# SKA-INAF/caesar-mrcnn

Measured on AMD Instinct MI355X. Metric: train images/sec (whole node) + detect ms/image, ResNet-101 256x256, higher is better.
Workload: dtype f32; 1 GPU; resnet101+FPN 256x256 3-class (+bg), nimg_per_gpu=4, train step (fwd+bwd+SGD), 512 train ROIs, 2000 proposals; global_batch=4, parallelism=dp1, weights=random init (Keras defaults)

## Files before the change

### caesar-mrcnn_amd/_hip.py

```python
import ctypes as C
import os
import threading

PKG_DIR = os.path.dirname(os.path.abspath(__file__))
LIB_PATH = os.path.join(PKG_DIR, "libmrcnn_hip.so")


class HipPathError(RuntimeError):
    pass


class ConvDesc(C.Structure):
    _fields_ = [(n, C.c_int32) for n in (
        "N", "H", "W", "Cin", "Cout", "KH", "KW", "stride", "pad_t", "pad_l", "OH", "OW",
        "act", "res_mode", "out_mode", "cmod")] + [
        ("out_n_stride", C.c_int64), ("out_h_stride", C.c_int64), ("out_w_stride", C.c_int64)]


class ConvProblem(C.Structure):
    _fields_ = [("d", ConvDesc)] + [(n, C.c_void_p) for n in ("x", "w", "bias", "scale", "shift", "res", "out", "z_out")]


class WgradProblem(C.Structure):
    _fields_ = [("d", ConvDesc), ("x", C.c_void_p), ("dy", C.c_void_p), ("dw", C.c_void_p), ("accumulate", C.c_int32)]
# ... 151 lines not shown
    "mrcnn_detection_targets": (C.c_int, [C.POINTER(DetTargetDesc)] + [_P] * 12),
    "mrcnn_conv2d_fwd_h16": (C.c_int, [C.POINTER(ConvDesc), C.c_int] + [_P] * 8),
    "mrcnn_conv2d_fwd_h16_res": (C.c_int, [C.POINTER(ConvDesc), C.c_int] + [_P] * 9),
    "mrcnn_conv2d_fwd_h16_supported": (C.c_int, [C.POINTER(ConvDesc), C.c_int]),
    "mrcnn_conv2d_dgrad_ep_h16": (C.c_int, [C.POINTER(ConvDesc), C.c_int, _P, _P, _P, _P, C.POINTER(BwdEpilogueH16), _P]),
    "mrcnn_conv2d_dgrad_ep": (C.c_int, [C.POINTER(ConvDesc), _P, _P, _P, _P, C.POINTER(BwdEpilogue), _P, C.c_size_t, _P]),
    "mrcnn_conv2d_wgrad_h16_workspace": (C.c_size_t, [C.POINTER(ConvDesc)]),
    "mrcnn_conv2d_wgrad_h16": (C.c_int, [C.POINTER(ConvDesc), C.c_int, _P, _P, _P, _P, C.c_size_t, C.c_int, C.c_float, _P]),
    "mrcnn_mask_out_fwd_h16": (C.c_int, [C.c_int, _P, _P, _P, _P, C.c_int64, C.c_int, C.c_int, _P]),
    "mrcnn_mask_out_bwd_h16": (C.c_int, [C.c_int] + [_P] * 8 + [C.c_int64, C.c_int, C.c_int, C.c_int, C.c_int, C.c_float, _P]),
    "mrcnn_weights_to_h16": (C.c_int, [_P, _P, _P, C.c_int, C.c_int, C.c_int, C.c_int, C.c_int, _P]),
    "mrcnn_weights_to_h16_batched": (C.c_int, [_P, _P, C.c_int, C.c_int, C.c_int, _P]),
    "mrcnn_cast_to_h16": (C.c_int, [_P, _P, C.c_int64, C.c_int, C.c_float, _P]),
    "mrcnn_epilogue_bwd_h16": (C.c_int, [C.c_int] + [_P] * 10 + [C.c_int64, C.c_int, C.c_int, C.c_float, _P]),
    "mrcnn_epilogue_bwd_h16_dy": (C.c_int, [C.c_int] + [_P] * 11 + [C.c_int64, C.c_int, C.c_int, C.c_float, _P]),
    "mrcnn_cast_from_h16": (C.c_int, [_P, _P, C.c_int64, C.c_int, C.c_float, _P]),
    "mrcnn_axpy_from_h16": (C.c_int, [_P, _P, C.c_int64, C.c_int, C.c_float, _P]),
    "mrcnn_rpn_targets_workspace": (C.c_size_t, [C.POINTER(RpnTargetDesc)]),
    "mrcnn_rpn_targets": (C.c_int, [C.POINTER(RpnTargetDesc)] + [_P] * 7 + [C.c_size_t, _P]),
    "mrcnn_detection_workspace": (C.c_size_t, [C.POINTER(DetectionDesc)]),
    "mrcnn_detection_fwd": (C.c_int, [C.POINTER(DetectionDesc)] + [_P] * 6 + [C.c_size_t, _P]),
    "mrcnn_losses_workspace": (C.c_size_t, [C.POINTER(LossDesc)]),
    "mrcnn_losses_fwd_bwd": (C.c_int, [C.POINTER(LossDesc)] + [_P] * 18 + [C.c_size_t, _P]),
    "mrcnn_grad_prepare": (C.c_int, [_P, _P, C.c_float, _P, C.c_int64, _P, _P]),
    "mrcnn_sumsq": (C.c_int, [_P, C.c_int64, _P, _P]),
    "mrcnn_sgd_momentum": (C.c_int, [_P, _P, _P, _P, C.c_float, C.c_float, C.c_float, _P, C.c_int64, _P]),
    "mrcnn_sgd_momentum_guarded": (C.c_int, [_P, _P, _P, _P, C.c_float, C.c_float, C.c_float, _P, C.c_int64, _P, _P]),
    "mrcnn_winograd_buffer_floats": (C.c_size_t, [C.c_int, C.c_int, C.c_int, C.c_int, C.c_int]),
    "mrcnn_winograd_weights": (C.c_int, [_P, _P, C.c_int, C.c_int, C.c_int, _P]),
    "mrcnn_gemm_batched_f32": (C.c_int, [_P, _P, _P, C.c_int, C.c_int, C.c_int, C.c_int, _P]),
    "mrcnn_winograd_gemm": (C.c_int, [_P, _P, _P, C.c_int, C.c_int, C.c_int, C.c_int, _P]),
    "mrcnn_winograd_group_floats": (C.c_size_t, [C.POINTER(WinoGroup), C.c_int, C.c_int]),
    "mrcnn_winograd_input_g": (C.c_int, [_P, _P, C.c_int, C.c_int, C.c_int, C.c_int, C.POINTER(WinoGroup), _P]),
    "mrcnn_winograd_weights_g": (C.c_int, [_P, _P, C.c_int, C.c_int, C.c_int, C.c_int, _P]),
    "mrcnn_winograd_output_g": (C.c_int, [_P, _P, _P, _P, _P, _P, C.c_int, C.c_int, C.c_int, C.c_int, C.c_int, C.POINTER(WinoGroup), _P]),
    "mrcnn_winograd_output_bwd_rows": (C.c_int, [C.POINTER(WinoGroup), C.c_int, C.c_int]),
    "mrcnn_winograd_output_bwd_g": (C.c_int, [_P] * 8 + [C.c_int, C.c_int, C.c_int, C.c_int, C.c_int, C.POINTER(WinoGroup), _P]),
    "mrcnn_winograd_output_bwd_zmask_g": (C.c_int, [_P] * 8 + [C.c_int, C.c_int, C.c_int, C.c_int, C.POINTER(WinoGroup), _P]),
    "mrcnn_winograd_output_bwd_sums": (C.c_int, [_P, C.c_int, C.c_int, _P, _P, _P, _P]),
    "mrcnn_winograd_dy_g": (C.c_int, [_P, _P, C.c_int, C.c_int, C.c_int, C.c_int, C.POINTER(WinoGroup), _P]),
    "mrcnn_winograd_dw_g": (C.c_int, [_P, _P, C.c_int, C.c_int, C.c_int, C.c_int, C.c_int, _P]),
    "mrcnn_deconv2x2_gemm": (C.c_int, [_P, _P, _P, _P, C.c_int, C.c_int, C.c_int, C.c_int, C.c_int, C.c_int, _P]),
    "mrcnn_allreduce_load": (C.c_int, [C.c_char_p]),
    "mrcnn_allreduce_unique_id": (C.c_int, [_P]),
    "mrcnn_allreduce_init": (C.c_int, [C.POINTER(_P), _P, C.c_int, C.c_int]),
    "mrcnn_allreduce_scratch": (C.c_size_t, [C.c_int, C.c_int64, C.c_int]),
    "mrcnn_allreduce_grad": (C.c_int, [_P, _P, C.c_int64, C.c_int64, C.c_int, _P, C.c_size_t, _P]),
    "mrcnn_allreduce_direct_plan": (C.c_int, [C.c_int, C.c_int, C.c_int64, C.c_int64, C.c_int, _P, _P, _P, _P]),
    "mrcnn_allreduce_direct_simulate": (C.c_int, [_P, _P, C.c_size_t, C.c_int, C.c_int64, C.c_int64, _P]),
    "mrcnn_allreduce_destroy": (C.c_int, [_P]),
    "mrcnn_allreduce_last_error": (C.c_char_p, []),
    "mrcnn_tuning_set": (C.c_int, [C.c_char_p, C.c_longlong]),
    "mrcnn_hip_version": (C.c_char_p, []),
}

_lib = None
_proxy = None
_tape = None
_tape_owner = None

_NO_RECORD = ("_workspace", "_fwd_plan", "_tiles_check", "_outline_check", "_draw_check", "_components_check", "_catalog_check", "_overview_check", "_planes_check", "_stats_check", "_gather_check", "_supported", "_status_offset", "_version", "mrcnn_allreduce_", "_scratch", "_floats", "_bwd_rows")


class _LibProxy(object):

    def __init__(self, real):
# ... 111 lines not shown
```

### caesar-mrcnn_amd/csrc/winograd.hip

```cpp
#include "common.h"
#include <type_traits>
#include <string.h>

template <int CV> struct WinoVec;
template <> struct WinoVec<4> { typedef f32x4 type; };
template <> struct WinoVec<2> { typedef float type __attribute__((ext_vector_type(2))); };

template <int OT, typename V> __device__ __forceinline__ void wino_bt(const V (&d)[OT + 2], V (&t)[OT + 2]) {
    if constexpr (OT == 2) {
        t[0] = d[0] - d[2];
        t[1] = d[1] + d[2];
        t[2] = d[2] - d[1];
        t[3] = d[1] - d[3];
    } else {
        const V a = d[4] - 4.f * d[2], b = d[3] - 4.f * d[1], c = d[4] - d[2], e = 2.f * (d[3] - d[1]);
        t[0] = 4.f * d[0] - 5.f * d[2] + d[4];
        t[1] = a + b;
        t[2] = a - b;
        t[3] = c + e;
        t[4] = c - e;
        t[5] = 4.f * d[1] - 5.f * d[3] + d[5];
    }
}
template <int OT, typename V> __device__ __forceinline__ void wino_at(const V (&m)[OT + 2], V (&y)[OT]) {
// ... 35 lines not shown
        u[0] = 0.25f * g[0];
        u[1] = (-1.f / 6.f) * (e + g[1]);
        u[2] = (-1.f / 6.f) * (e - g[1]);
        const float f = (1.f / 24.f) * g[0] + (1.f / 6.f) * g[2], h = (1.f / 12.f) * g[1];
        u[3] = f + h;
        u[4] = f - h;
        u[5] = g[2];
    }
}
template <int OT> __device__ __forceinline__ void wino_gt(const float (&u)[OT + 2], float (&w)[3]) {
    if constexpr (OT == 2) {
        w[0] = u[0] + 0.5f * (u[1] + u[2]);
        w[1] = 0.5f * (u[1] - u[2]);
        w[2] = 0.5f * (u[1] + u[2]) + u[3];
    } else {
        const float p = u[1] + u[2], q = u[3] + u[4];
        w[0] = 0.25f * u[0] - (1.f / 6.f) * p + (1.f / 24.f) * q;
        w[1] = (1.f / 6.f) * (u[2] - u[1]) + (1.f / 12.f) * (u[3] - u[4]);
        w[2] = (1.f / 6.f) * (q - p) + u[5];
    }
}

struct WinoGrp { int th_n, tw_n, oh0, ow0; };
struct WinoTile { int n, th, tw; };
__device__ __forceinline__ WinoTile wino_tile(long long t, int th_n, int tw_n) {
    WinoTile r;
    r.tw = (int)(t % tw_n);
    const long long q = t / tw_n;
    r.th = (int)(q % th_n);
    r.n = (int)(q / th_n);
    return r;
}

template <int OTH, int OTW, int CV>
__global__ __launch_bounds__(256) void winograd_input_kernel(const float* __restrict__ x, float* __restrict__ V, int N, int H, int W,
                                                             int C, long long T, long long Tp, const WinoGrp g) {
    typedef typename WinoVec<CV>::type vec;
    constexpr int ITH = OTH + 2, ITW = OTW + 2;
    const int cn = C / CV;
    const long long i = (long long)blockIdx.x * 256 + threadIdx.x;
    if (i >= T * cn) return;
    const long long t = i / cn;
    const int c = (int)(i - t * cn) * CV;
    const WinoTile q = wino_tile(t, g.th_n, g.tw_n);
    const int ih0 = g.oh0 + OTH * q.th - 1, iw0 = g.ow0 + OTW * q.tw - 1;
    vec tt[ITH][ITW];
#pragma unroll
    for (int s = 0; s < ITW; ++s) {
        vec col[ITH], o[ITH];
#pragma unroll
        for (int r = 0; r < ITH; ++r) {
            const int ih = ih0 + r, iw = iw0 + s;
            vec val = {};
            if ((unsigned)ih < (unsigned)H && (unsigned)iw < (unsigned)W) val = *(const vec*)(x + (((long long)q.n * H + ih) * W + iw) * C + c);
            col[r] = val;
        }
        wino_bt<OTH>(col, o);
#pragma unroll
        for (int r = 0; r < ITH; ++r) tt[r][s] = o[r];
    }
#pragma unroll
    for (int r = 0; r < ITH; ++r) {
        vec v[ITW];
        wino_bt<OTW>(tt[r], v);
#pragma unroll
        for (int s = 0; s < ITW; ++s) *(vec*)(V + ((long long)(r * ITW + s) * Tp + t) * C + c) = v[s];
    }
}

template <int OTH, int OTW>
__global__ __launch_bounds__(256) void winograd_weight_kernel(const float* __restrict__ g, float* __restrict__ U, int Cin, int Cout) {
    constexpr int ITH = OTH + 2, ITW = OTW + 2;
    const long long i = (long long)blockIdx.x * 256 + threadIdx.x;
    const long long n = (long long)Cin * Cout;
    if (i >= n) return;
    float t[ITH][3];
#pragma unroll
    for (int b = 0; b < 3; ++b) {
        float col[3], o[ITH];
#pragma unroll
        for (int a = 0; a < 3; ++a) col[a] = g[(long long)(a * 3 + b) * n + i];
        wino_g<OTH>(col, o);
#pragma unroll
        for (int a = 0; a < ITH; ++a) t[a][b] = o[a];
    }
#pragma unroll
    for (int a = 0; a < ITH; ++a) {
        float u[ITW];
        wino_g<OTW>(t[a], u);
#pragma unroll
        for (int b = 0; b < ITW; ++b) U[(long long)(a * ITW + b) * n + i] = u[b];
    }
}

template <int OTH, int OTW, int CV>
__device__ __forceinline__ void wino_output_tile(const float* __restrict__ Mt, float* __restrict__ out, float* __restrict__ z,
                                                 const typename WinoVec<CV>::type bi, const typename WinoVec<CV>::type sc,
                                                 const typename WinoVec<CV>::type sh, int H, int W, int C, long long Tp, int act,
                                                 const WinoGrp& g, long long t, int c) {
    typedef typename WinoVec<CV>::type vec;
    constexpr int ITH = OTH + 2, ITW = OTW + 2;
    const WinoTile q = wino_tile(t, g.th_n, g.tw_n);
    vec s[OTH][ITW];
#pragma unroll
    for (int k = 0; k < ITW; ++k) {
        vec col[ITH], o[OTH];
#pragma unroll
        for (int r = 0; r < ITH; ++r) col[r] = *(const vec*)(Mt + ((long long)(r * ITW + k) * Tp + t) * C + c);
        wino_at<OTH>(col, o);
#pragma unroll
        for (int a = 0; a < OTH; ++a) s[a][k] = o[a];
    }
#pragma unroll
    for (int a = 0; a < OTH; ++a) {
        vec y[OTW];
        wino_at<OTW>(s[a], y);
        const int oh = g.oh0 + OTH * q.th + a;
        if (oh >= H) continue;
#pragma unroll
        for (int b = 0; b < OTW; ++b) {
            const int ow = g.ow0 + OTW * q.tw + b;
            if (ow >= W) continue;
            const long long addr = (((long long)q.n * H + oh) * W + ow) * C + c;
            vec zv, o;
#pragma unroll
            for (int e = 0; e < CV; ++e) {
                zv[e] = y[b][e] + bi[e];
                float v = sc[e] * zv[e] + sh[e];
                if (act == MRCNN_ACT_RELU) v = fmaxf(v, 0.f);
                o[e] = v;
            }
            if (z) *(vec*)(z + addr) = zv;
            *(vec*)(out + addr) = o;
        }
    }
}

template <int OTH, int OTW, int CV>
__global__ __launch_bounds__(256) void winograd_output_kernel(const float* __restrict__ Mt, float* __restrict__ out, float* __restrict__ z,
                                                              const float* __restrict__ bias, const float* __restrict__ scale,
                                                              const float* __restrict__ shift, int N, int H, int W, int C, long long T,
                                                              long long Tp, int act, const WinoGrp g) {
    typedef typename WinoVec<CV>::type vec;
    const int cn = C / CV;
    const long long i = (long long)blockIdx.x * 256 + threadIdx.x;
    if (i >= T * cn) return;
    const long long t = i / cn;
    const int c = (int)(i - t * cn) * CV;
    vec bi = {}, sc, sh = {};
#pragma unroll
    for (int e = 0; e < CV; ++e) sc[e] = 1.f;
    if (bias) bi = *(const vec*)(bias + c);
    if (scale) { sc = *(const vec*)(scale + c); sh = *(const vec*)(shift + c); }
    wino_output_tile<OTH, OTW, CV>(Mt, out, z, bi, sc, sh, H, W, C, Tp, act, g, t, c);
}

template <int CV>
__device__ __forceinline__ typename WinoVec<CV>::type wino_buffer_load(__amdgpu_buffer_rsrc_t rsrc, unsigned voff, unsigned soff) {
    typename WinoVec<CV>::type r;
    if constexpr (CV == 2) {
        const auto v = __builtin_amdgcn_raw_buffer_load_b64(rsrc, (int)voff, (int)soff, 0);
        r[0] = __uint_as_float(v[0]); r[1] = __uint_as_float(v[1]);
    } else {
        const auto v = __builtin_amdgcn_raw_buffer_load_b128(rsrc, (int)voff, (int)soff, 0);
        r[0] = __uint_as_float(v[0]); r[1] = __uint_as_float(v[1]); r[2] = __uint_as_float(v[2]); r[3] = __uint_as_float(v[3]);
    }
// ... 367 lines not shown
static inline long long wino_grp_tiles(const mrcnn_wino_group* g, int N) { return (long long)N * g->th_n * g->tw_n; }
static inline int wino_grp_nb(const mrcnn_wino_group* g) { return (g->oth + 2) * (g->otw + 2); }
static inline int wino_grp_cv(const mrcnn_wino_group* g) { return g->oth == 2 && g->otw == 2 ? 4 : 2; }

#define WINO_LAUNCH_G(kernel, g, grid4, grid2, ...)                                                                          \
    do {                                                                                                                     \
        if ((g)->oth == 2 && (g)->otw == 2) hipLaunchKernelGGL((kernel<2, 2, 4>), grid4, dim3(256), 0, (hipStream_t)stream, __VA_ARGS__); \
        else if ((g)->oth == 4 && (g)->otw == 4) hipLaunchKernelGGL((kernel<4, 4, 2>), grid2, dim3(256), 0, (hipStream_t)stream, __VA_ARGS__); \
        else if ((g)->oth == 4) hipLaunchKernelGGL((kernel<4, 2, 2>), grid2, dim3(256), 0, (hipStream_t)stream, __VA_ARGS__); \
        else hipLaunchKernelGGL((kernel<2, 4, 2>), grid2, dim3(256), 0, (hipStream_t)stream, __VA_ARGS__);                  \
    } while (0)
#define WINO_LAUNCH_W(kernel, oth, otw, grid, ...)                                                                           \
    do {                                                                                                                     \
        if ((oth) == 2 && (otw) == 2) hipLaunchKernelGGL((kernel<2, 2>), grid, dim3(256), 0, (hipStream_t)stream, __VA_ARGS__); \
        else if ((oth) == 4 && (otw) == 4) hipLaunchKernelGGL((kernel<4, 4>), grid, dim3(256), 0, (hipStream_t)stream, __VA_ARGS__); \
        else if ((oth) == 4) hipLaunchKernelGGL((kernel<4, 2>), grid, dim3(256), 0, (hipStream_t)stream, __VA_ARGS__);     \
        else hipLaunchKernelGGL((kernel<2, 4>), grid, dim3(256), 0, (hipStream_t)stream, __VA_ARGS__);                     \
    } while (0)

extern "C" size_t mrcnn_winograd_group_floats(const mrcnn_wino_group* g, int N, int C) {
    if (!g || N <= 0 || C <= 0 || (g->oth != 2 && g->oth != 4) || (g->otw != 2 && g->otw != 4) || g->th_n <= 0 || g->tw_n <= 0) return 0;
    return (size_t)wino_grp_nb(g) * (size_t)wino_rows(wino_grp_tiles(g, N)) * (size_t)C;
}

extern "C" int mrcnn_winograd_input_g(const float* x, float* V, int N, int H, int W, int C, const mrcnn_wino_group* g, void* stream) {
    if (!x || !V || !wino_grp_ok(g, N, H, W, C)) return MRCNN_ERR_ARG;
    const long long T = wino_grp_tiles(g, N);
    const WinoGrp k = {g->th_n, g->tw_n, g->oh0, g->ow0};
    const dim3 g4((unsigned)cdiv64(T * C / 4, 256)), g2((unsigned)cdiv64(T * C / 2, 256));
    WINO_LAUNCH_G(winograd_input_kernel, g, g4, g2, x, V, N, H, W, C, T, wino_rows(T), k);
    return mrcnn_launch_status();
}

extern "C" int mrcnn_winograd_weights_g(const float* w, float* U, int Cin, int Cout, int oth, int otw, void* stream) {
    if (!w || !U || Cin <= 0 || Cout <= 0 || (oth != 2 && oth != 4) || (otw != 2 && otw != 4)) return MRCNN_ERR_ARG;
    const dim3 grid((unsigned)cdiv64((long long)Cin * Cout, 256));
    WINO_LAUNCH_W(winograd_weight_kernel, oth, otw, grid, w, U, Cin, Cout);
    return mrcnn_launch_status();
}

extern "C" int mrcnn_winograd_output_g(const float* Mt, float* out, float* z, const float* bias, const float* scale, const float* shift,
                                       int N, int H, int W, int C, int act, const mrcnn_wino_group* g, void* stream) {
    if (!Mt || !out || !wino_grp_ok(g, N, H, W, C) || (scale && !shift)) return MRCNN_ERR_ARG;
    if (act != MRCNN_ACT_NONE && act != MRCNN_ACT_RELU) return MRCNN_ERR_UNSUPPORTED;
    const long long T = wino_grp_tiles(g, N);
    const WinoGrp k = {g->th_n, g->tw_n, g->oh0, g->ow0};
    const dim3 g4((unsigned)cdiv64(T * C / 4, 256)), g2((unsigned)cdiv64(T * C / 2, 256));
    WINO_LAUNCH_G(winograd_output_kernel, g, g4, g2, Mt, out, z, bias, scale, shift, N, H, W, C, T, wino_rows(T), act, k);
    return mrcnn_launch_status();
}

static int wino_bwd_lanes_lg(const mrcnn_wino_group* g, int C) {
    const int cn = C / wino_grp_cv(g);
    if (cn <= 0 || cn > 256 || (cn & (cn - 1)) || cn * wino_grp_cv(g) != C) return -1;
    int lg = 0;
    while ((1 << lg) < cn) ++lg;
    return lg;
}
extern "C" int mrcnn_winograd_output_bwd_rows(const mrcnn_wino_group* g, int N, int C) {
    if (!g || N <= 0 || (g->oth != 2 && g->oth != 4) || (g->otw != 2 && g->otw != 4) || g->th_n <= 0 || g->tw_n <= 0) return 0;
    const int lg = wino_bwd_lanes_lg(g, C);
    if (lg < 0) return 0;
    const long long T = wino_grp_tiles(g, N), R = 256 >> lg, cap = 4LL * mrcnn_num_cus();
    const long long wgs = cdiv64(T, R);
    return (int)(wgs < cap ? wgs : cap);
}

template <int MASK>
static int wino_output_bwd_launch(const float* Mt, float* dz_below, const float* below_out, const float* below_z, const float* scale,
                                  const float* mean, const float* rstd, const float* fwd_shift, float* partials, int N, int H, int W,
                                  int C, const mrcnn_wino_group* g, void* stream) {
    const int lg = wino_bwd_lanes_lg(g, C);
    const long long T = wino_grp_tiles(g, N);
    if (lg < 0) return MRCNN_ERR_UNSUPPORTED;
    if ((long long)wino_grp_nb(g) * wino_rows(T) * C * 4 >= (1LL << 32) || (long long)N * H * W * C * 4 >= (1LL << 32)) return MRCNN_ERR_UNSUPPORTED;
    const dim3 grid((unsigned)mrcnn_winograd_output_bwd_rows(g, N, C));
// ... 112 lines not shown
```

### caesar-mrcnn_amd/engine.py

```python
import collections
import contextlib
import gc
import operator
from functools import partial
import os
import numpy as np
import torch

from . import ops
from . import _hip as _hip_mod
from ._hip import ACT_NONE, ACT_RELU, ACT_SIGMOID, RES_NONE, RES_SAME, RES_UP2
from .params import ParamLayout, deconv_gemm_to_keras, deconv_keras_to_gemm, granule_coefficients, init_weights

H16_WIDE_LAYERS = ("fpn_p2", "fpn_p3", "fpn_p4", "fpn_p5", "rpn_conv_shared", "mrcnn_class_conv1", "mrcnn_class_conv2")

LOSS_NAMES = ("rpn_class_loss", "rpn_bbox_loss", "mrcnn_class_loss", "mrcnn_bbox_loss", "mrcnn_mask_loss")


DIRECT, WINO, H16 = "direct", "winograd", "h16"
Ctx = collections.namedtuple("Ctx", "x z out act path V", defaults=(DIRECT, None))
BlockCtx = collections.namedtuple("BlockCtx", "a b c shortcut h16")


_on = lambda s: s != "0"

SWITCHES = (
    ("head_dtype", None, None, None, "ti"),
    ("sparse_mask_bwd", None, True, None, "t"),
    ("h16_wide", "MRCNN_H16_WIDE", True, _on, "ti"),
    ("h16_blocks", "MRCNN_H16_BLOCKS", True, _on, "ti"),
    ("h16_all_blocks", "MRCNN_H16_ALL_BLOCKS", True, _on, "ti"),
    ("h16_fused_bwd", "MRCNN_H16_FUSED_BWD", True, _on, "t"),
    ("h16_roialign", "MRCNN_H16_ROIALIGN", True, _on, "ti"),
    ("h16_phase_bwd", "MRCNN_H16_PHASE_BWD", True, _on, "t"),
    ("winograd", "MRCNN_WINOGRAD", True, _on, "ti"),
    ("winograd_wgrad", "MRCNN_WINOGRAD_WGRAD", True, _on, "t"),
    ("trunk_winograd", "MRCNN_WINOGRAD_TRUNK", True, _on, "ti"),
    ("trunk_winograd_min_rows", "MRCNN_WINOGRAD_TRUNK_MIN_ROWS", 4096, int, "ti"),
    ("infer_mask_tile", "MRCNN_WINOGRAD_INFER_MASK_TILE", 4, int, "i"),
    ("sk16_infer", "MRCNN_SK16_INFER", True, _on, "i"),
    ("fused_mask_out_bwd", None, True, None, "t"),
    ("fused_dgrad_epilogue", None, True, None, "t"),
    ("gather_roialign_bwd", "MRCNN_GATHER_ROIALIGN_BWD", True, _on, "t"),
    ("multi_launch", "MRCNN_MULTI_LAUNCH", True, _on, "ti"),
    ("wgrad_prio", "MRCNN_WGRAD_PRIO", 0, int, ""),
    ("aux_prio", "MRCNN_AUX_PRIO", 0, int, ""),
)
_TRAIN_SWITCHES = operator.attrgetter(*(s[0] for s in SWITCHES if "t" in s[4]))
_INFER_SWITCHES = operator.attrgetter(*(s[0] for s in SWITCHES if "i" in s[4]))
_INFER_CFG = operator.attrgetter("PRE_NMS_LIMIT", "POST_NMS_ROIS_INFERENCE", "RPN_NMS_THRESHOLD", "DETECTION_MAX_INSTANCES",
                                 "DETECTION_MIN_CONFIDENCE", "DETECTION_NMS_THRESHOLD")


@contextlib.contextmanager
def _capture(graph):
    gc.collect()
    was = gc.isenabled()
    gc.disable()
    try:
        with torch.cuda.graph(graph):
            yield
    finally:
        if was:
            gc.enable()


@contextlib.contextmanager
def _tuning(key, value, restore, on=True):
    if on:
        ops.tuning_set(key, value)
    try:
        yield
    finally:
        if on:
            ops.tuning_set(key, restore)
# ... 354 lines not shown
                return got
        d = self._h16_dgrad(op, dz)
        return ops.epilogue_bwd_h16(d, y if act != ACT_NONE else None, z, below.scale, below.mean, below.rstd, below.dgamma,
                                    below.dbeta, below.db, act, 1.0 / S)

    def _block_bwd_h16(self, blk, d16, ctxs, S):
        ca, cb, cc, c1c = ctxs.a, ctxs.b, ctxs.c, ctxs.shortcut
        c2a, c2b, c2c = blk.c2a, blk.c2b, blk.c2c
        dzc, dy = ops.epilogue_bwd_h16(d16, cc.out, cc.z, c2c.scale, c2c.mean, c2c.rstd, c2c.dgamma, c2c.dbeta, c2c.db, ACT_RELU,
                                       1.0 / S, want_dy=True)
        self._h16_wgrad(c2c, cc.x, dzc, S)
        dzb = self._h16_dgrad_ep(c2c, dzc, c2b, cb, S)
        self._h16_wgrad(c2b, cb.x, dzb, S)
        dza = self._h16_dgrad_ep(c2b, dzb, c2a, ca, S)
        self._h16_wgrad(c2a, ca.x, dza, S)
        if blk.c1 is None:
            return self._h16_dgrad(c2a, dza, dx_res=dy)
        x16 = ca.x
        N, H, W, C = x16.shape
        st = c2a.stride
        dz1 = self._h16_bwd(blk.c1, dy, c1c, S, need_dx=False)
        dx = ops.empty((N, H, W, C), x16.dtype, x16.device)
        strides = None
        if st != 1:
            ops.fill_zero(dx)
            strides = (H * W * C, st * W * C, st * C)
        self._h16_dgrad(blk.c1, dz1, out=dx, out_strides=strides)
        self._h16_dgrad(c2a, dza, dx_res=dx, out=dx, out_strides=strides)
        return dx

    def _S(self):
        return float(self.loss_scale) if self.head_dtype == torch.float16 else 1.0

    def _wino_fwd(self, op, x, act, train, infer_tile=2):
        out = ops.empty(tuple(x.shape[:3]) + (op.wshape[3],), torch.float32, x.device)
        z = ops.empty_like(out) if (train and op.bn) else None
        V = ops.empty((ops.winograd_v_floats(tuple(x.shape)),), torch.float32, x.device) if (train and self.winograd_wgrad) else None
        ops.conv2d_winograd(x, self._wino_U(op, 0, x.shape, train, infer_tile), op.b, op.scale, op.shift, act, out=out, z_out=z, keep_v=V)
        return out, (Ctx(x, z, out, act, WINO, V) if train else None)

    def _forward_multi(self, layers, xs, act=ACT_NONE, train=False):
        if self.trunk_winograd and any(self._wino_trunk_ok(op, x.shape) for op, x in zip(layers, xs)):
            res = [None] * len(layers)
            rest = []
            for i, (op, x) in enumerate(zip(layers, xs)):
                if self._wino_trunk_ok(op, x.shape):
                    res[i] = self._wino_fwd(op, x, act, train)
                else:
                    rest.append(i)
            if rest:
                sub = self._forward_multi([layers[i] for i in rest], [xs[i] for i in rest], act, train) if len(rest) > 1 else \
                    [layers[rest[0]].forward(xs[rest[0]], act, train=train)]
                for i, r in zip(rest, sub):
                    res[i] = r
            return res
        if self.multi_launch and 1 < len(layers) <= 5:
            probs, zs = [], []
            for op, x in zip(layers, xs):
                d = ops.conv_desc(tuple(x.shape), op.wshape, op.stride, op.padding, act)
                out = ops.empty((d.N, d.OH, d.OW, d.Cout), torch.float32, x.device)
                z = ops.empty_like(out) if (train and op.bn) else None
                zs.append(z)
                probs.append(dict(x=x, w=op.w, bias=op.b, scale=op.scale, shift=op.shift, stride=op.stride,
                                  padding=op.padding, act=act, out=out, z_out=z))
            outs = ops.conv2d_multi(probs)
            if outs is not None:
                return [(o, Ctx(x, z, o, act) if train else None) for o, x, z in zip(outs, xs, zs)]
        return [op.forward(x, act, train=train) for op, x in zip(layers, xs)]

    def _dgrad_multi(self, layers, dzs, ctxs, outs=None, accumulate=False):
        outs = list(outs) if outs is not None else [None] * len(layers)
        accs = list(accumulate) if isinstance(accumulate, (list, tuple)) else [accumulate] * len(layers)
# ... 219 lines not shown
            p16h = None
        if p16h is not None:
            x16 = ops.roialign_h16(rois, p16h, cfg.POOL_SIZE, image_area).view(B * R, cfg.POOL_SIZE, cfg.POOL_SIZE, -1)
        else:
            pooled = ops.roialign(rois, fms, cfg.POOL_SIZE, image_area)
            x = pooled.view(B * R, cfg.POOL_SIZE, cfg.POOL_SIZE, -1)
        if h16:
            self._ensure_h16()
            if p16h is None:
                x16 = ops.cast_to_h16(x, self.head_dtype)
            h1, c1 = self._h16_fwd(self.op("mrcnn_class_conv1"), x16, ACT_RELU, train)
            h2_16, c2 = self._h16_fwd(self.op("mrcnn_class_conv2"), h1, ACT_RELU, train)
            h2 = ops.cast_from_h16(h2_16)
        else:
            h1, c1 = self.op("mrcnn_class_conv1").forward(x, ACT_RELU, train=train)
            h2, c2 = self.op("mrcnn_class_conv2").forward(h1, ACT_RELU, train=train)
        lg, c3 = self.op("mrcnn_class_logits").forward(h2, train=train)
        bb, c4 = self.op("mrcnn_bbox_fc").forward(h2, train=train)
        logits = lg.view(B, R, cfg.NUM_CLASSES)
        probs = ops.softmax_rows(logits)
        return logits, probs, bb.view(B, R, cfg.NUM_CLASSES, 4), (c1, c2, c3, c4)

    def _mask_head_fwd(self, rois, fms, p16h, image_area, train):
        cfg = self.cfg
        B, R = rois.shape[0], rois.shape[1]
        if p16h is not None:
            x = None
            x16 = ops.roialign_h16(rois, p16h, cfg.MASK_POOL_SIZE, image_area).view(B * R, cfg.MASK_POOL_SIZE, cfg.MASK_POOL_SIZE, -1)
        else:
            pooled = ops.roialign(rois, fms, cfg.MASK_POOL_SIZE, image_area)
            x = pooled.view(B * R, cfg.MASK_POOL_SIZE, cfg.MASK_POOL_SIZE, -1)
        ctxs = []
        if self.head_dtype is None:
            for i in range(1, 5):
                op = self.op("mrcnn_mask_conv%d" % i)
                if self._wino_ok(op, x.shape):
                    x, c = self._wino_fwd(op, x, ACT_RELU, train, self.infer_mask_tile)
                else:
                    x, c = op.forward(x, ACT_RELU, train=train)
                ctxs.append(c)
        else:
            self._ensure_h16()
            h = x16 if p16h is not None else ops.cast_to_h16(x, self.head_dtype)
            for i in range(1, 5):
                h, c = self._h16_fwd(self.op("mrcnn_mask_conv%d" % i), h, ACT_RELU, train)
                ctxs.append(c)
            dc, mop = self.op("mrcnn_mask_deconv"), self.op("mrcnn_mask")
            Cd = dc.wshape[3] // 4
            C_ = mop.wshape[3]
            if Cd % 256 == 0 and C_ <= 16:
                up = ops.deconv2x2_h16(h, self._h16[dc.name][0], dc.b, Cd, ACT_RELU)
                m = ops.mask_out_fwd_h16(up, mop.w.view(mop.wshape[2], C_), mop.b)
                ctxs.append(Ctx(h, None, up, ACT_RELU, H16) if train else None)
                ctxs.append(Ctx(up, None, m, ACT_SIGMOID, H16) if train else None)
                return m.view(B, R, m.shape[1], m.shape[2], m.shape[3]), ctxs
            x = ops.cast_from_h16(h)
        dc = self.op("mrcnn_mask_deconv")
        up = ops.deconv2x2(x, dc.w.view(dc.wshape[2], dc.wshape[3]), dc.b, ACT_RELU)
        m, cm = self.op("mrcnn_mask").forward(up, ACT_SIGMOID, train=train)
        ctxs.append(Ctx(x, None, up, ACT_RELU) if train else None)
        ctxs.append(cm)
        return m.view(B, R, m.shape[1], m.shape[2], m.shape[3]), ctxs

    def infer(self, images, windows_norm):
        cfg = self.cfg
        B, H, W = images.shape[0], images.shape[1], images.shape[2]
        area = float(H * W)
        with _tuning("sk16", 1 if self.sk16_infer else 0, 0):
            pyr, p16, p16h, _ = self._trunk_fwd(images, False)
            _, rpn_probs, rpn_bbox, _ = self._rpn_fwd(pyr, p16, False)
# ... 143 lines not shown

    def _mask_head_bwd_rows(self, g, ctxs, rois, dP, area, before_adjoint):
        cfg = self.cfg
        c1, c2, c3, c4, cdec, cm = ctxs
        mop, dc = self.op("mrcnn_mask"), self.op("mrcnn_mask_deconv")
        x_in, up = cdec.x, cdec.out
        C_ = cm.out.shape[-1]
        S = self._S()
        wgrad = lambda launch, *operands: self._fork(self.wgrad_stream, launch, *operands)
        d16 = None
        if cdec.path == H16:
            dzg = ops.mask_out_bwd_h16(g, cm.out, up, mop.w.view(mop.wshape[2], mop.wshape[3]),
                                       mop.dw.view(mop.wshape[2], mop.wshape[3]), mop.db, dc.db, S)
            wgrad(partial(ops.conv2d_wgrad_h16, x_in, dzg, dc.wshape, 1, "same", dw=dc.dw, multiplier=1.0 / S), x_in, dzg)
            d16 = ops.conv2d_h16(dzg, self._h16[dc.name][1], (1, 1, dc.wshape[3], dc.wshape[2]), None, None, None, 1, "valid",
                                 ACT_NONE)
        elif self.fused_mask_out_bwd and C_ <= 16 and up.shape[-1] % 64 == 0 and up.shape[-1] <= 1024:
            dzg = ops.mask_out_bwd(g, cm.out, up, mop.w.view(mop.wshape[2], mop.wshape[3]),
                                   mop.dw.view(mop.wshape[2], mop.wshape[3]), mop.db, dc.db)
        else:
            dz, _ = mop.epilogue_bwd(g, cm)
            mop.wgrad(dz, cm)
            d_up = mop.dgrad(dz, cm)
            dzu = ops.empty_like(d_up)
            ops.epilogue_bwd(d_up, up, None, None, None, None, None, dzu, None, None, dc.db, ACT_RELU)
            dzg = ops.pixel_unshuffle2(dzu)
        if d16 is None:
            wgrad(partial(ops.conv2d_wgrad, x_in, dzg, dc.wshape, 1, "valid", dw=dc.dw), x_in, dzg)
        chain = [(self.op("mrcnn_mask_conv%d" % i), c) for i, c in ((4, c4), (3, c3), (2, c2), (1, c1))]
        if c4.path != H16:
            dz = self._dgrad_ep(dzg, dc.wt, "valid", chain[0][0], chain[0][1])
            for k, (op, c) in enumerate(chain):
                if c.V is not None:
                    wgrad(partial(ops.conv2d_wgrad_winograd, c.V, tuple(c.x.shape), dz, op.dw), c.V, dz)
                else:
                    wgrad(partial(ops.conv2d_wgrad, c.x, dz, op.wshape, op.stride, op.padding, dw=op.dw), c.x, dz)
                wino = c.path == WINO
                if k + 1 < len(chain):
                    below, bctx = chain[k + 1]
                    if wino and self.fused_dgrad_epilogue and below.bn is not None:
                        dz = ops.conv2d_dgrad_ep_winograd(dz, self._wino_U(op, 1, dz.shape), bctx.out if bctx.act != ACT_NONE else None,
                                                          bctx.z, below.scale, below.mean, below.rstd, below.dgamma, below.dbeta,
                                                          below.db, bctx.act, fwd_shift=below.shift)
                    elif wino:
                        dz = below.epilogue_bwd(ops.conv2d_winograd(dz, self._wino_U(op, 1, dz.shape)), bctx)[0]
                    else:
                        dz = self._dgrad_ep(dz, op.wt, op.dgrad_padding, below, bctx)
                elif wino:
                    d = ops.conv2d_winograd(dz, self._wino_U(op, 1, dz.shape))
                else:
                    d = op.dgrad(dz, c)
        else:
            if d16 is None:
                d = ops.conv2d(dzg, dc.wt, stride=1, padding="valid")
                d16 = ops.cast_to_h16(d, self.head_dtype, multiplier=S)
            for op, c in chain:
                d16 = self._h16_bwd(op, d16, c, S)
            d = None if self.h16_roialign else ops.cast_from_h16(d16, 1.0 / S)
        B, R = rois.shape[0], rois.shape[1]
        _hip_mod.ev_wait(torch.cuda.current_stream(self.dev), before_adjoint)
        if d is None:
            ops.roialign_bwd_h16(rois, d16.view(B, R, cfg.MASK_POOL_SIZE, cfg.MASK_POOL_SIZE, -1), dP, cfg.MASK_POOL_SIZE, area, 1.0 / S)
            return
        ops.roialign_bwd(rois, d.view(B, R, cfg.MASK_POOL_SIZE, cfg.MASK_POOL_SIZE, -1), dP, cfg.MASK_POOL_SIZE, area)

    def _dgrad_ep(self, dz, wt, padding, below, below_ctx):
        z, out, act = below_ctx.z, below_ctx.out, below_ctx.act
        if self.fused_dgrad_epilogue and below.bn is not None:
            got = ops.conv2d_dgrad_ep(dz, wt, padding, out if act != ACT_NONE else None, z, below.scale, below.mean, below.rstd,
                                      below.dgamma, below.dbeta, below.db, act)
            if got is not None:
                return got
# ... 300 lines not shown
```

### caesar-mrcnn_amd/ops.py

```python
import ctypes as C
import math
import os

import torch

from . import _hip
from ._hip import (ACT_NONE, ACT_RELU, ACT_SIGMOID, OUT_DECONV2, OUT_NHWC, RES_NONE, RES_SAME, RES_UP2,
                   check, current_stream, ptr)

BN_EPS = 1e-3


def _need_cuda(*ts):
    for t in ts:
        if t is not None and not t.is_cuda:
            raise _hip.HipPathError("hot-path operators need device tensors (got a CPU tensor)")
        if t is not None and not t.is_contiguous():
            raise _hip.HipPathError("hot-path operators need contiguous tensors")


def same_padding(size, k, stride):
    out = -(-size // stride)
    total = max((out - 1) * stride + k - size, 0)
    return out, total // 2


def conv_desc(x_shape, w_shape, stride=1, padding="same", act=ACT_NONE, res_mode=RES_NONE):
    N, H, W, Cin = x_shape
    KH, KW, wcin, Cout = w_shape
    assert wcin == Cin, (x_shape, w_shape)
    d = _hip.ConvDesc()
    d.N, d.H, d.W, d.Cin, d.Cout, d.KH, d.KW, d.stride = N, H, W, Cin, Cout, KH, KW, stride
# ... 1597 lines not shown
    return 2 if nb == 16 else 4


def winograd_ok(xshape, wshape, stride=1, padding="same", min_rows=None):
    N, H, W, Cin = xshape
    kh, kw, cin, cout = wshape
    if min_rows is None:
        min_rows = _WINO_MIN_ROWS
    return (kh == 3 and kw == 3 and stride == 1 and padding in ("same", (1, 1)) and H % 2 == 0 and W % 2 == 0 and cin == Cin and
            Cin % 16 == 0 and cout % 128 == 0 and N * H * W >= min_rows and N * (H // 2) * (W // 2) * 16 * max(Cin, cout) < 2 ** 31)


def winograd_weights(w, out=None, tile=2):
    kh, kw, cin, cout = w.shape
    assert kh == 3 and kw == 3 and w.is_contiguous()
    if tile != TILE_MIXED:
        _need_cuda(w, out)
        nb = (tile + 2) ** 2
        if out is None:
            out = torch.empty((nb, cin, cout), dtype=torch.float32, device=w.device)
        assert out.shape[0] == nb
        check(_hip.lib().mrcnn_winograd_weights(ptr(w), ptr(out), cin, cout, tile, current_stream()), "mrcnn_winograd_weights")
        return out
    shapes = ((4, 4), (4, 2), (2, 4), (2, 2))
    if out is None:
        out = [torch.empty(((a + 2) * (b + 2), cin, cout), dtype=torch.float32, device=w.device) for a, b in shapes]
    _need_cuda(w, *out)
    for (a, b), u in zip(shapes, out):
        assert u.shape[0] == (a + 2) * (b + 2)
        check(_hip.lib().mrcnn_winograd_weights_g(ptr(w), ptr(u), cin, cout, a, b, current_stream()), "mrcnn_winograd_weights_g")
    return out


def _winograd_run(x, U, finish, keep_v=None, after_input=None):
    N, H, W, Cin = x.shape
    tile = _wino_tile_of(U)
    Us = U if isinstance(U, (list, tuple)) else [U]
    cout = Us[0].shape[2]
    groups = winograd_groups(H, W, tile)
    lib = _hip.lib()
    nvs = [lib.mrcnn_winograd_group_floats(C.byref(g), N, Cin) for g in groups]
    nms = [lib.mrcnn_winograd_group_floats(C.byref(g), N, cout) for g in groups]
    nv = sum(nvs)
    V = keep_v if keep_v is not None else workspace(nv * 4, x.device, "winograd_v")[:nv * 4].view(torch.float32)
    assert keep_v is None or (keep_v.numel() == nv and keep_v.dtype == torch.float32)
    Mt = workspace(max(nms) * 4, x.device, "winograd_m")
    off = 0
    for gi, (g, u) in enumerate(zip(groups, Us)):
        Vg = V[off:off + nvs[gi]]
        off += nvs[gi]
        check(lib.mrcnn_winograd_input_g(ptr(x), ptr(Vg), N, H, W, Cin, C.byref(g), current_stream()), "mrcnn_winograd_input_g")
        if gi == 0 and after_input is not None:
            after_input()
        nb = _wino_nb(g)
        rows = nvs[gi] // (nb * Cin)
        check(lib.mrcnn_winograd_gemm(ptr(Vg), ptr(u), ptr(Mt), nb, rows, Cin, cout, current_stream()), "mrcnn_winograd_gemm")
        finish(g, Mt)


def winograd_v_floats(xshape, tile=None):
    N, H, W, Cin = xshape
    if tile is None:
        tile = winograd_tile(xshape)
    lib = _hip.lib()
    return sum(lib.mrcnn_winograd_group_floats(C.byref(g), N, Cin) for g in winograd_groups(H, W, tile))


def conv2d_winograd(x, U, bias=None, scale=None, shift=None, act=ACT_NONE, out=None, z_out=None, keep_v=None, after_input=None):
    _need_cuda(x, bias, scale, shift, out, z_out, keep_v)
    N, H, W, _ = x.shape
    cout = (U[0] if isinstance(U, (list, tuple)) else U).shape[2]
    if out is None:
        out = empty((N, H, W, cout), torch.float32, x.device)
    lib = _hip.lib()

    def finish(g, Mt):
        check(lib.mrcnn_winograd_output_g(ptr(Mt), ptr(out), ptr(z_out), ptr(bias), ptr(scale), ptr(shift), N, H, W, cout, act, C.byref(g),
                                          current_stream()), "mrcnn_winograd_output_g")

    _winograd_run(x, U, finish, keep_v, after_input)
    return out


def conv2d_dgrad_ep_winograd(dz, Ut, below_out, below_z, scale, mean, rstd, dgamma, dbeta, dbias, act, fwd_shift=None):
    _need_cuda(dz, below_out, below_z, scale, mean, rstd, dgamma, dbeta, dbias, fwd_shift)
    N, H, W, _ = dz.shape
    cout = (Ut[0] if isinstance(Ut, (list, tuple)) else Ut).shape[2]
    out = empty((N, H, W, cout), torch.float32, dz.device)
    lib = _hip.lib()
    zmask = act == ACT_RELU and fwd_shift is not None and below_z is not None and scale is not None
    if dgamma is None:
        mean = rstd = None
    want_sums = dgamma is not None or dbeta is not None or dbias is not None
    rows = [lib.mrcnn_winograd_output_bwd_rows(C.byref(g), N, cout) for g in winograd_groups(H, W, _wino_tile_of(Ut))]
    assert min(rows) > 0, "channel count does not fit the Winograd data-gradient transform"
    part = ptr(workspace(sum(rows) * 3 * cout * 4, dz.device, "winograd_bwd_sums")) if want_sums else None
    done = []

    def finish(g, Mt):
        p = None
        if want_sums:
            p = part + sum(done) * 3 * cout * 4
            done.append(rows[len(done)])
        if zmask:
            check(lib.mrcnn_winograd_output_bwd_zmask_g(ptr(Mt), ptr(out), ptr(below_z), ptr(scale), ptr(fwd_shift), ptr(mean), ptr(rstd),
                                                        p, N, H, W, cout, C.byref(g), current_stream()),
# ... 193 lines not shown
```

### include/mrcnn_hip.h

```cpp
#ifndef MRCNN_HIP_H
#define MRCNN_HIP_H

#include <stddef.h>
#include <stdint.h>

#ifdef __cplusplus
extern "C" {
#endif

#define MRCNN_OK 0
#define MRCNN_ERR_ARG (-1)
#define MRCNN_ERR_LAUNCH (-2)
#define MRCNN_ERR_WORKSPACE (-3)
#define MRCNN_ERR_UNSUPPORTED (-4)

#define MRCNN_ACT_NONE 0
#define MRCNN_ACT_RELU 1
#define MRCNN_ACT_SIGMOID 2

#define MRCNN_RES_NONE 0
#define MRCNN_RES_SAME 1
#define MRCNN_RES_UP2 2

#define MRCNN_OUT_NHWC 0
// ... 360 lines not shown
    int32_t mask_loss_dice;
    float w[5];
} mrcnn_loss_desc;
size_t mrcnn_losses_workspace(const mrcnn_loss_desc* d);
int mrcnn_losses_fwd_bwd(const mrcnn_loss_desc* d, const int32_t* rpn_match, const float* rpn_bbox_t,
                         const float* rpn_class_logits, const float* rpn_bbox,
                         const int32_t* target_class_ids, const float* target_bbox,
                         const float* target_mask, const int32_t* active_class_ids,
                         const float* mrcnn_class_logits, const float* mrcnn_bbox,
                         const float* mrcnn_mask, float* losses, float* d_rpn_class_logits,
                         float* d_rpn_bbox, float* d_mrcnn_class_logits, float* d_mrcnn_bbox,
                         float* d_mrcnn_mask, void* workspace, size_t workspace_bytes, void* stream);

int mrcnn_grad_prepare(float* grads, const float* params, float grad_scale, const float* gran_coef,
                       int64_t n, float* sumsq_out, void* stream);
int mrcnn_sumsq(const float* g, int64_t n, float* out_scalar, void* stream);
int mrcnn_sgd_momentum(float* params, float* momentum_buf, const float* grads, const float* sumsq,
                       float clipnorm, float lr, float momentum, const float* gran_coef, int64_t n,
                       void* stream);
int mrcnn_sgd_momentum_guarded(float* params, float* momentum_buf, const float* grads, const float* sumsq,
                               float clipnorm, float lr, float momentum, const float* gran_coef, int64_t n,
                               unsigned* skipped_steps, void* stream);

typedef struct mrcnn_wino_group {
    int oth, otw;
    int th_n, tw_n;
    int oh0, ow0;
} mrcnn_wino_group;
size_t mrcnn_winograd_group_floats(const mrcnn_wino_group* g, int N, int C);
size_t mrcnn_winograd_buffer_floats(int N, int H, int W, int C, int tile);
int mrcnn_winograd_weights(const float* w_hwio, float* U, int Cin, int Cout, int tile, void* stream);
int mrcnn_winograd_weights_g(const float* w_hwio, float* U, int Cin, int Cout, int oth, int otw, void* stream);
int mrcnn_winograd_input_g(const float* x, float* V, int N, int H, int W, int C, const mrcnn_wino_group* g, void* stream);
int mrcnn_gemm_batched_f32(const float* V, const float* U, float* Mt, int nb, int rows, int K, int Cout, void* stream);
int mrcnn_winograd_gemm(const float* V, const float* U, float* Mt, int nb, int rows, int K, int Cout, void* stream);
int mrcnn_winograd_output_g(const float* Mt, float* out, float* z_out, const float* bias, const float* scale, const float* shift,
                            int N, int H, int W, int C, int act, const mrcnn_wino_group* g, void* stream);
int mrcnn_winograd_output_bwd_rows(const mrcnn_wino_group* g, int N, int C);
int mrcnn_winograd_output_bwd_g(const float* Mt, float* dz_below, const float* below_out, const float* below_z, const float* scale,
                                const float* mean, const float* rstd, float* partials, int N, int H, int W, int C, int act,
                                const mrcnn_wino_group* g, void* stream);
int mrcnn_winograd_output_bwd_zmask_g(const float* Mt, float* dz_below, const float* below_z, const float* scale, const float* shift,
                                      const float* mean, const float* rstd, float* partials, int N, int H, int W, int C,
                                      const mrcnn_wino_group* g, void* stream);
int mrcnn_winograd_output_bwd_sums(const float* partials, int rows, int C, float* dgamma, float* dbeta, float* dbias, void* stream);
int mrcnn_winograd_dy_g(const float* dy, float* dM, int N, int H, int W, int C, const mrcnn_wino_group* g, void* stream);
int mrcnn_winograd_dw_g(const float* dU, float* dw_hwio, int Cin, int Cout, int accumulate, int oth, int otw, void* stream);

int mrcnn_deconv2x2_gemm(const float* x, const float* w_gemm, const float* bias, float* out, int N, int H, int W, int Cin, int Cd,
                         int act, void* stream);

#define MRCNN_UNIQUE_ID_BYTES 128
#define MRCNN_ALLREDUCE_RCCL 0
#define MRCNN_ALLREDUCE_DIRECT 1
int mrcnn_allreduce_load(const char* librccl_path);
int mrcnn_allreduce_unique_id(void* id_128_bytes);
int mrcnn_allreduce_init(void** comm, const void* id_128_bytes, int rank, int world);
size_t mrcnn_allreduce_scratch(int world, int64_t max_range_floats, int algo);
int mrcnn_allreduce_grad(void* comm, float* grads, int64_t start, int64_t end, int algo, float* scratch,
                         size_t scratch_bytes, void* stream);
int mrcnn_allreduce_direct_plan(int world, int rank, int64_t start, int64_t end, int phase, int64_t* plan, int64_t* own_off,
                                int64_t* own_len, int64_t* slot_stride);
int mrcnn_allreduce_direct_simulate(float* const* grads, float* const* scratch, size_t scratch_bytes, int world, int64_t start,
                                    int64_t end, void* stream);
int mrcnn_allreduce_destroy(void* comm);
const char* mrcnn_allreduce_last_error(void);
// ... 19 lines not shown
```

Before: 115.7 images/s.

## Feed mask-head Winograd convs from pre-activation z, skipping activated output stores

Adds a Winograd input-transform kernel that applies the BN scale/shift and ReLU on the fly while reading the previous layer's pre-activation z. The mask-head conv chain then skips writing the activated output tensor when the next layer is also Winograd. The backward pass already uses z with a zero mask, and the weight gradient uses the saved V. This removes one full-size activation write and its later reread per mask conv in training. The cost is recomputing the affine and ReLU on every tile read (halo elements are read more than once) and extra asserts and coupling between forward and backward paths.

```diff
diff --git a/caesar-mrcnn_amd/_hip.py b/caesar-mrcnn_amd/_hip.py
--- a/caesar-mrcnn_amd/_hip.py
+++ b/caesar-mrcnn_amd/_hip.py
@@ -207,6 +207,7 @@
     "mrcnn_winograd_gemm": (C.c_int, [_P, _P, _P, C.c_int, C.c_int, C.c_int, C.c_int, _P]),
     "mrcnn_winograd_group_floats": (C.c_size_t, [C.POINTER(WinoGroup), C.c_int, C.c_int]),
     "mrcnn_winograd_input_g": (C.c_int, [_P, _P, C.c_int, C.c_int, C.c_int, C.c_int, C.POINTER(WinoGroup), _P]),
+    "mrcnn_winograd_input_act_g": (C.c_int, [_P, _P, _P, C.c_int, _P, C.c_int, C.c_int, C.c_int, C.c_int, C.POINTER(WinoGroup), _P]),
     "mrcnn_winograd_weights_g": (C.c_int, [_P, _P, C.c_int, C.c_int, C.c_int, C.c_int, _P]),
     "mrcnn_winograd_output_g": (C.c_int, [_P, _P, _P, _P, _P, _P, C.c_int, C.c_int, C.c_int, C.c_int, C.c_int, C.POINTER(WinoGroup), _P]),
     "mrcnn_winograd_output_bwd_rows": (C.c_int, [C.POINTER(WinoGroup), C.c_int, C.c_int]),
diff --git a/caesar-mrcnn_amd/csrc/winograd.hip b/caesar-mrcnn_amd/csrc/winograd.hip
--- a/caesar-mrcnn_amd/csrc/winograd.hip
+++ b/caesar-mrcnn_amd/csrc/winograd.hip
@@ -91,40 +91,77 @@
     return r;
 }
 
+template <int OTH, int OTW, int CV, bool ZSRC>
+__device__ __forceinline__ void wino_input_tile(const float* __restrict__ x, float* __restrict__ V, const typename WinoVec<CV>::type sc,
+                                                const typename WinoVec<CV>::type sh, int act, int H, int W, int C, long long Tp,
+                                                const WinoGrp& g, long long t, int c) {
+    typedef typename WinoVec<CV>::type vec;
+    constexpr int ITH = OTH + 2, ITW = OTW + 2;
+    const WinoTile q = wino_tile(t, g.th_n, g.tw_n);
+    const int ih0 = g.oh0 + OTH * q.th - 1, iw0 = g.ow0 + OTW * q.tw - 1;
+    vec tt[ITH][ITW];
+#pragma unroll
+    for (int s = 0; s < ITW; ++s) {
+        vec col[ITH], o[ITH];
+        bool in[ITH];
+#pragma unroll
+        for (int r = 0; r < ITH; ++r) {
+            const int ih = ih0 + r, iw = iw0 + s;
+            vec val = {};
+            in[r] = (unsigned)ih < (unsigned)H && (unsigned)iw < (unsigned)W;
+            if (in[r]) val = *(const vec*)(x + (((long long)q.n * H + ih) * W + iw) * C + c);
+            col[r] = val;
+        }
+        if constexpr (ZSRC) {
+#pragma unroll
+            for (int r = 0; r < ITH; ++r)
+#pragma unroll
+                for (int e = 0; e < CV; ++e) {
+                    float v = sc[e] * col[r][e] + sh[e];
+                    if (act == MRCNN_ACT_RELU) v = fmaxf(v, 0.f);
+                    col[r][e] = in[r] ? v : 0.f;
+                }
+        }
+        wino_bt<OTH>(col, o);
+#pragma unroll
+        for (int r = 0; r < ITH; ++r) tt[r][s] = o[r];
+    }
+#pragma unroll
+    for (int r = 0; r < ITH; ++r) {
+        vec v[ITW];
+        wino_bt<OTW>(tt[r], v);
+#pragma unroll
+        for (int s = 0; s < ITW; ++s) *(vec*)(V + ((long long)(r * ITW + s) * Tp + t) * C + c) = v[s];
+    }
+}
+
 template <int OTH, int OTW, int CV>
 __global__ __launch_bounds__(256) void winograd_input_kernel(const float* __restrict__ x, float* __restrict__ V, int N, int H, int W,
                                                              int C, long long T, long long Tp, const WinoGrp g) {
     typedef typename WinoVec<CV>::type vec;
-    constexpr int ITH = OTH + 2, ITW = OTW + 2;
     const int cn = C / CV;
     const long long i = (long long)blockIdx.x * 256 + threadIdx.x;
     if (i >= T * cn) return;
     const long long t = i / cn;
     const int c = (int)(i - t * cn) * CV;
-    const WinoTile q = wino_tile(t, g.th_n, g.tw_n);
-    const int ih0 = g.oh0 + OTH * q.th - 1, iw0 = g.ow0 + OTW * q.tw - 1;
-    vec tt[ITH][ITW];
-#pragma unroll
-    for (int s = 0; s < ITW; ++s) {
-        vec col[ITH], o[ITH];
-#pragma unroll
-        for (int r = 0; r < ITH; ++r) {
-            const int ih = ih0 + r, iw = iw0 + s;
-            vec val = {};
-            if ((unsigned)ih < (unsigned)H && (unsigned)iw < (unsigned)W) val = *(const vec*)(x + (((long long)q.n * H + ih) * W + iw) * C + c);
-            col[r] = val;
-        }
-        wino_bt<OTH>(col, o);
-#pragma unroll
-        for (int r = 0; r < ITH; ++r) tt[r][s] = o[r];
-    }
-#pragma unroll
-    for (int r = 0; r < ITH; ++r) {
-        vec v[ITW];
-        wino_bt<OTW>(tt[r], v);
-#pragma unroll
-        for (int s = 0; s < ITW; ++s) *(vec*)(V + ((long long)(r * ITW + s) * Tp + t) * C + c) = v[s];
-    }
+    wino_input_tile<OTH, OTW, CV, false>(x, V, vec{}, vec{}, MRCNN_ACT_NONE, H, W, C, Tp, g, t, c);
+}
+
+template <int OTH, int OTW, int CV>
+__global__ __launch_bounds__(256) void winograd_input_act_kernel(const float* __restrict__ z, const float* __restrict__ scale,
+                                                                 const float* __restrict__ shift, int act, float* __restrict__ V, int N,
+                                                                 int H, int W, int C, long long T, long long Tp, const WinoGrp g) {
+    typedef typename WinoVec<CV>::type vec;
+    const int cn = C / CV;
+    const long long i = (long long)blockIdx.x * 256 + threadIdx.x;
+    if (i >= T * cn) return;
+    const long long t = i / cn;
+    const int c = (int)(i - t * cn) * CV;
+    vec sc, sh = {};
+#pragma unroll
+    for (int e = 0; e < CV; ++e) sc[e] = 1.f;
+    if (scale) { sc = *(const vec*)(scale + c); sh = *(const vec*)(shift + c); }
+    wino_input_tile<OTH, OTW, CV, true>(z, V, sc, sh, act, H, W, C, Tp, g, t, c);
 }
 
 template <int OTH, int OTW>
@@ -190,7 +227,7 @@
                 o[e] = v;
             }
             if (z) *(vec*)(z + addr) = zv;
-            *(vec*)(out + addr) = o;
+            if (out) *(vec*)(out + addr) = o;
         }
     }
 }
@@ -624,6 +661,17 @@
     return mrcnn_launch_status();
 }
 
+extern "C" int mrcnn_winograd_input_act_g(const float* z, const float* scale, const float* shift, int act, float* V, int N, int H, int W,
+                                          int C, const mrcnn_wino_group* g, void* stream) {
+    if (!z || !V || !wino_grp_ok(g, N, H, W, C) || (scale && !shift)) return MRCNN_ERR_ARG;
+    if (act != MRCNN_ACT_NONE && act != MRCNN_ACT_RELU) return MRCNN_ERR_UNSUPPORTED;
+    const long long T = wino_grp_tiles(g, N);
+    const WinoGrp k = {g->th_n, g->tw_n, g->oh0, g->ow0};
+    const dim3 g4((unsigned)cdiv64(T * C / 4, 256)), g2((unsigned)cdiv64(T * C / 2, 256));
+    WINO_LAUNCH_G(winograd_input_act_kernel, g, g4, g2, z, scale, shift, act, V, N, H, W, C, T, wino_rows(T), k);
+    return mrcnn_launch_status();
+}
+
 extern "C" int mrcnn_winograd_weights_g(const float* w, float* U, int Cin, int Cout, int oth, int otw, void* stream) {
     if (!w || !U || Cin <= 0 || Cout <= 0 || (oth != 2 && oth != 4) || (otw != 2 && otw != 4)) return MRCNN_ERR_ARG;
     const dim3 grid((unsigned)cdiv64((long long)Cin * Cout, 256));
@@ -633,7 +681,7 @@
 
 extern "C" int mrcnn_winograd_output_g(const float* Mt, float* out, float* z, const float* bias, const float* scale, const float* shift,
                                        int N, int H, int W, int C, int act, const mrcnn_wino_group* g, void* stream) {
-    if (!Mt || !out || !wino_grp_ok(g, N, H, W, C) || (scale && !shift)) return MRCNN_ERR_ARG;
+    if (!Mt || (!out && !z) || !wino_grp_ok(g, N, H, W, C) || (scale && !shift)) return MRCNN_ERR_ARG;
     if (act != MRCNN_ACT_NONE && act != MRCNN_ACT_RELU) return MRCNN_ERR_UNSUPPORTED;
     const long long T = wino_grp_tiles(g, N);
     const WinoGrp k = {g->th_n, g->tw_n, g->oh0, g->ow0};
diff --git a/caesar-mrcnn_amd/engine.py b/caesar-mrcnn_amd/engine.py
--- a/caesar-mrcnn_amd/engine.py
+++ b/caesar-mrcnn_amd/engine.py
@@ -41,6 +41,7 @@
     ("sk16_infer", "MRCNN_SK16_INFER", True, _on, "i"),
     ("fused_mask_out_bwd", None, True, None, "t"),
     ("fused_dgrad_epilogue", None, True, None, "t"),
+    ("winograd_zsource", None, True, None, "t"),
     ("gather_roialign_bwd", "MRCNN_GATHER_ROIALIGN_BWD", True, _on, "t"),
     ("multi_launch", "MRCNN_MULTI_LAUNCH", True, _on, "ti"),
     ("wgrad_prio", "MRCNN_WGRAD_PRIO", 0, int, ""),
@@ -461,12 +462,16 @@
     def _S(self):
         return float(self.loss_scale) if self.head_dtype == torch.float16 else 1.0
 
-    def _wino_fwd(self, op, x, act, train, infer_tile=2):
-        out = ops.empty(tuple(x.shape[:3]) + (op.wshape[3],), torch.float32, x.device)
-        z = ops.empty_like(out) if (train and op.bn) else None
-        V = ops.empty((ops.winograd_v_floats(tuple(x.shape)),), torch.float32, x.device) if (train and self.winograd_wgrad) else None
-        ops.conv2d_winograd(x, self._wino_U(op, 0, x.shape, train, infer_tile), op.b, op.scale, op.shift, act, out=out, z_out=z, keep_v=V)
-        return out, (Ctx(x, z, out, act, WINO, V) if train else None)
+    def _wino_fwd(self, op, x, act, train, infer_tile=2, store_out=True):
+        xt = x.z if isinstance(x, ops.ZSource) else x
+        oshape = tuple(xt.shape[:3]) + (op.wshape[3],)
+        out = ops.empty(oshape, torch.float32, xt.device) if store_out else None
+        z = ops.empty(oshape, torch.float32, xt.device) if (train and op.bn) else None
+        V = ops.empty((ops.winograd_v_floats(tuple(xt.shape)),), torch.float32, xt.device) if (train and self.winograd_wgrad) else None
+        assert xt is x or V is not None, "a layer fed from z keeps V: its weight gradient has no other input"
+        ops.conv2d_winograd(x, self._wino_U(op, 0, xt.shape, train, infer_tile), op.b, op.scale, op.shift, act, out=out, z_out=z, keep_v=V,
+                            store_out=store_out)
+        return out, (Ctx(x if xt is x else None, z, out, act, WINO, V) if train else None)
 
     def _forward_multi(self, layers, xs, act=ACT_NONE, train=False):
         if self.trunk_winograd and any(self._wino_trunk_ok(op, x.shape) for op, x in zip(layers, xs)):
@@ -752,10 +757,15 @@
             x = pooled.view(B * R, cfg.MASK_POOL_SIZE, cfg.MASK_POOL_SIZE, -1)
         ctxs = []
         if self.head_dtype is None:
-            for i in range(1, 5):
-                op = self.op("mrcnn_mask_conv%d" % i)
-                if self._wino_ok(op, x.shape):
-                    x, c = self._wino_fwd(op, x, ACT_RELU, train, self.infer_mask_tile)
+            mops = [self.op("mrcnn_mask_conv%d" % i) for i in range(1, 5)]
+            wino = [self._wino_ok(op, tuple(x.shape[:3]) + (mops[k - 1].wshape[3] if k else x.shape[3],)) for k, op in enumerate(mops)]
+            hand_on = [train and self.winograd_zsource and self.winograd_wgrad and self.fused_dgrad_epilogue and wino[k] and
+                       k + 1 < len(mops) and wino[k + 1] and op.bn is not None and op.scale is not None and op.shift is not None
+                       for k, op in enumerate(mops)]
+            for k, op in enumerate(mops):
+                if wino[k]:
+                    out, c = self._wino_fwd(op, x, ACT_RELU, train, self.infer_mask_tile, store_out=not hand_on[k])
+                    x = ops.ZSource(c.z, op.scale, op.shift, ACT_RELU) if hand_on[k] else out
                 else:
                     x, c = op.forward(x, ACT_RELU, train=train)
                 ctxs.append(c)
@@ -965,12 +975,16 @@
             dz = self._dgrad_ep(dzg, dc.wt, "valid", chain[0][0], chain[0][1])
             for k, (op, c) in enumerate(chain):
                 if c.V is not None:
-                    wgrad(partial(ops.conv2d_wgrad_winograd, c.V, tuple(c.x.shape), dz, op.dw), c.V, dz)
+                    wgrad(partial(ops.conv2d_wgrad_winograd, c.V, tuple(dz.shape[:3]) + (op.wshape[2],), dz, op.dw), c.V, dz)
                 else:
                     wgrad(partial(ops.conv2d_wgrad, c.x, dz, op.wshape, op.stride, op.padding, dw=op.dw), c.x, dz)
                 wino = c.path == WINO
                 if k + 1 < len(chain):
                     below, bctx = chain[k + 1]
+                    assert bctx.out is not None or bctx.act == ACT_NONE or (
+                        wino and self.fused_dgrad_epilogue and below.bn is not None and bctx.act == ACT_RELU and
+                        bctx.z is not None and below.scale is not None and below.shift is not None), \
+                        "%s stored no activated output, and this data gradient would read it" % below.name
                     if wino and self.fused_dgrad_epilogue and below.bn is not None:
                         dz = ops.conv2d_dgrad_ep_winograd(dz, self._wino_U(op, 1, dz.shape), bctx.out if bctx.act != ACT_NONE else None,
                                                           bctx.z, below.scale, below.mean, below.rstd, below.dgamma, below.dbeta,
diff --git a/caesar-mrcnn_amd/ops.py b/caesar-mrcnn_amd/ops.py
--- a/caesar-mrcnn_amd/ops.py
+++ b/caesar-mrcnn_amd/ops.py
@@ -1,3 +1,4 @@
+import collections
 import ctypes as C
 import math
 import os
@@ -1661,7 +1662,13 @@
     return out
 
 
+ZSource = collections.namedtuple("ZSource", "z scale shift act")
+
+
 def _winograd_run(x, U, finish, keep_v=None, after_input=None):
+    src = x if isinstance(x, ZSource) else None
+    if src is not None:
+        x = src.z
     N, H, W, Cin = x.shape
     tile = _wino_tile_of(U)
     Us = U if isinstance(U, (list, tuple)) else [U]
@@ -1678,7 +1685,11 @@
     for gi, (g, u) in enumerate(zip(groups, Us)):
         Vg = V[off:off + nvs[gi]]
         off += nvs[gi]
-        check(lib.mrcnn_winograd_input_g(ptr(x), ptr(Vg), N, H, W, Cin, C.byref(g), current_stream()), "mrcnn_winograd_input_g")
+        if src is None:
+            check(lib.mrcnn_winograd_input_g(ptr(x), ptr(Vg), N, H, W, Cin, C.byref(g), current_stream()), "mrcnn_winograd_input_g")
+        else:
+            check(lib.mrcnn_winograd_input_act_g(ptr(x), ptr(src.scale), ptr(src.shift), src.act, ptr(Vg), N, H, W, Cin, C.byref(g),
+                                                 current_stream()), "mrcnn_winograd_input_act_g")
         if gi == 0 and after_input is not None:
             after_input()
         nb = _wino_nb(g)
@@ -1695,12 +1706,16 @@
     return sum(lib.mrcnn_winograd_group_floats(C.byref(g), N, Cin) for g in winograd_groups(H, W, tile))
 
 
-def conv2d_winograd(x, U, bias=None, scale=None, shift=None, act=ACT_NONE, out=None, z_out=None, keep_v=None, after_input=None):
-    _need_cuda(x, bias, scale, shift, out, z_out, keep_v)
-    N, H, W, _ = x.shape
+def conv2d_winograd(x, U, bias=None, scale=None, shift=None, act=ACT_NONE, out=None, z_out=None, keep_v=None, after_input=None,
+                    store_out=True):
+    xt = x.z if isinstance(x, ZSource) else x
+    _need_cuda(xt, bias, scale, shift, out, z_out, keep_v, *(x[1:3] if isinstance(x, ZSource) else ()))
+    N, H, W, _ = xt.shape
     cout = (U[0] if isinstance(U, (list, tuple)) else U).shape[2]
-    if out is None:
-        out = empty((N, H, W, cout), torch.float32, x.device)
+    if not store_out:
+        assert out is None and z_out is not None, "store_out=False keeps z_out only"
+    elif out is None:
+        out = empty((N, H, W, cout), torch.float32, xt.device)
     lib = _hip.lib()
 
     def finish(g, Mt):
diff --git a/include/mrcnn_hip.h b/include/mrcnn_hip.h
--- a/include/mrcnn_hip.h
+++ b/include/mrcnn_hip.h
@@ -416,6 +416,8 @@
 int mrcnn_winograd_weights(const float* w_hwio, float* U, int Cin, int Cout, int tile, void* stream);
 int mrcnn_winograd_weights_g(const float* w_hwio, float* U, int Cin, int Cout, int oth, int otw, void* stream);
 int mrcnn_winograd_input_g(const float* x, float* V, int N, int H, int W, int C, const mrcnn_wino_group* g, void* stream);
+int mrcnn_winograd_input_act_g(const float* z, const float* scale, const float* shift, int act, float* V, int N, int H, int W, int C,
+                               const mrcnn_wino_group* g, void* stream);
 int mrcnn_gemm_batched_f32(const float* V, const float* U, float* Mt, int nb, int rows, int K, int Cout, void* stream);
 int mrcnn_winograd_gemm(const float* V, const float* U, float* Mt, int nb, int rows, int K, int Cout, void* stream);
 int mrcnn_winograd_output_g(const float* Mt, float* out, float* z_out, const float* bias, const float* scale, const float* shift,
```

Measured after the change: 116.3 images/s (median of 6 runs). Within noise of the previous version (+0.5%).
